# GewelsJI/MVLT

Hardware: AMD Instinct MI355X
Metric: image-text pairs/sec/node, PVT-tiny MVLT pre-train step (higher is better)
Workload: dtype bf16

## Files before the change

### mvlt_amd/_lib.py

```python
import ctypes as C
import os

import torch

_HERE = os.path.dirname(os.path.abspath(__file__))
LIB_PATH = os.environ.get("MVLT_HIP_LIB") or os.path.join(_HERE, "libmvlt_hip.so")


class MVLTError(RuntimeError):
    pass


if not os.path.exists(LIB_PATH):
    raise ImportError(f"{LIB_PATH} is missing: build it with `python -m mvlt_amd.build` (hipcc, gfx950). "
                      "mvlt_amd has no CPU or eager fallback.")
lib = C.CDLL(LIB_PATH)

c_int, c_float, c_void_p, c_long = C.c_int, C.c_float, C.c_void_p, C.c_long


class RowMap(C.Structure):
    _fields_ = [(n, c_int) for n in ("mode", "rows_per_batch", "batch_stride", "offset",
                                     "r", "w_in", "tokens_in", "hw_out", "w_out", "c_seg", "h_in")]

# ... 225 lines not shown

PLAN_VERSION = 3
_plan_sizes = [(n, getattr(lib, n + "_sizeof")(), C.sizeof(c)) for n, c in PLAN_STRUCTS]
if lib.mvlt_plan_version() != PLAN_VERSION or any(have != want for _, have, want in _plan_sizes):
    raise ImportError(f"plan entry points mismatch: {LIB_PATH} is version {lib.mvlt_plan_version()}, the binding is version {PLAN_VERSION}; (struct, bytes in the library, "
                      f"bytes in the binding): {_plan_sizes} (stale build? run python -m mvlt_amd.build)")

OPT_PROTOTYPES = {
    "mvlt_opt_version": (_i, []),
    "mvlt_adamw_step_groups": (_i, [_vp, _vp, _vp, _vp, _vp, _l, _vp, _vp, _vp, _i, _vp, _vp, _vp]),
}
for _name, (_res, _args) in OPT_PROTOTYPES.items():
    if not hasattr(lib, _name):
        raise ImportError(f"{LIB_PATH} does not export {_name} (include/mvlt_hip_opt.h): stale build? run python -m mvlt_amd.build")
    _fn = getattr(lib, _name)
    _fn.restype, _fn.argtypes = _res, _args

OPT_VERSION = 1
if lib.mvlt_opt_version() != OPT_VERSION:
    raise ImportError(f"optimizer entry points mismatch: {LIB_PATH} is version {lib.mvlt_opt_version()}, the binding is version {OPT_VERSION} (stale build? run python -m mvlt_amd.build)")

LAMB_PROTOTYPES = {
    "mvlt_lamb_version": (_i, []),
    "mvlt_lamb_check_tables": (_i, [_vp, _i, _vp, _i, _l, _i]),
    "mvlt_lamb_moments": (_i, [_vp, _vp, _vp, _vp, _l, _vp, _vp, _i, _vp, _i, _vp, _i, _vp, _vp, _vp, _vp]),
    "mvlt_lamb_fold": (_i, [_vp, _i, _vp, _i, _vp, _i, _i, _vp, _vp, _vp]),
    "mvlt_lamb_apply": (_i, [_vp, _vp, _vp, _vp, _l, _vp, _vp, _i, _vp, _i, _vp, _i, _vp, _vp, _vp]),
}
for _name, (_res, _args) in LAMB_PROTOTYPES.items():
    if not hasattr(lib, _name):
        raise ImportError(f"{LIB_PATH} does not export {_name} (include/mvlt_hip_lamb.h): stale build? run python -m mvlt_amd.build")
    _fn = getattr(lib, _name)
    _fn.restype, _fn.argtypes = _res, _args

LAMB_VERSION = 1
if lib.mvlt_lamb_version() != LAMB_VERSION:
    raise ImportError(f"LAMB entry points mismatch: {LIB_PATH} is version {lib.mvlt_lamb_version()}, the binding is version {LAMB_VERSION} (stale build? run python -m mvlt_amd.build)")

LOSS_PROTOTYPES = {
    "mvlt_loss_version": (_i, []),
    "mvlt_ce_smooth_fwd": (_i, [_vp, _vp, _l, _f, _vp, _vp, _vp, _vp, _i, _i, _i, _i, _vp]),
    "mvlt_ce_smooth_bwd": (_i, [_vp, _vp, _l, _f, _vp, _vp, _vp, _vp, _vp, _i, _i, _i, _i, _i, _i, _vp]),
}
for _name, (_res, _args) in LOSS_PROTOTYPES.items():
    if not hasattr(lib, _name):
        raise ImportError(f"{LIB_PATH} does not export {_name} (include/mvlt_hip_loss.h): stale build? run python -m mvlt_amd.build")
    _fn = getattr(lib, _name)
    _fn.restype, _fn.argtypes = _res, _args

LOSS_VERSION = 1
if lib.mvlt_loss_version() != LOSS_VERSION:
    raise ImportError(f"loss entry points mismatch: {LIB_PATH} is version {lib.mvlt_loss_version()}, the binding is version {LOSS_VERSION} (stale build? run python -m mvlt_amd.build)")

DT = {torch.bfloat16: 0, torch.float32: 1}


def last_kernel():
    s = lib.mvlt_last_kernel().decode()
    s = s.replace("(anonymous namespace)::", "")
    if s.startswith("void "):
        s = s[5:]
    depth = 0
    for i, ch in enumerate(s):
        depth += ch == "<"
        depth -= ch == ">"
        if ch == "(" and depth == 0:
            return s[:i]
    return s


def check(rc, what):
    if rc != 0:
        raise MVLTError(f"{what} failed ({rc}): {lib.mvlt_last_error().decode()}")


_raw_stream, _cur_device = torch._C._cuda_getCurrentRawStream, torch._C._cuda_getDevice


def stream_ptr():
    return _raw_stream(_cur_device())


def ptr(t):
    if t is None:
        return None
    if not t.is_cuda:
        raise MVLTError("mvlt_amd ops need CUDA/HIP tensors (no CPU fallback)")
    return t.data_ptr()


def rowmap(rows_per_batch=0, batch_stride=0, offset=0):
    return RowMap(0, rows_per_batch, batch_stride, offset, 0, 0, 0, 0, 0, 0, 0)


def patchmap(r, w_in, tokens_in, hw_out, w_out, c_seg):
    return RowMap(1, 0, 0, 0, r, w_in, tokens_in, hw_out, w_out, c_seg, 0)


def conv3map(h, w, tokens_in, c_seg):
    return RowMap(2, 0, 0, 0, 3, w, tokens_in, h * w, w, c_seg, h)
```

### mvlt_amd/build.py

```python
import concurrent.futures
import os
import subprocess
import sys

HERE = os.path.dirname(os.path.abspath(__file__))
CSRC = os.path.join(HERE, "csrc")
OBJ = os.path.join(HERE, "csrc", "_obj")
LIB = os.path.join(HERE, "libmvlt_hip.so")
ARCH = "gfx950"
FLAGS = ["--offload-arch=" + ARCH, "-O3", "-std=c++17", "-fPIC", "-ffp-contract=fast", "-Wno-unused-result"]
EXTRA = {f: ["-fno-slp-vectorize"] for f in ("mlp_fused.hip", "mlp_pipe.hip", "mlp_wgrad.hip")}


def _sources():
    return sorted(f for f in os.listdir(CSRC) if f.endswith(".hip"))


def source_hash():
    import hashlib
    h = hashlib.sha256()
    files = sorted(os.path.join(CSRC, f) for f in os.listdir(CSRC) if f.endswith((".hip", ".h", ".inc")))
    files += [os.path.join(HERE, "..", "include", h) for h in ("mvlt_hip.h", "mvlt_hip_ext.h", "mvlt_hip_ema.h", "mvlt_hip_plan.h", "mvlt_hip_opt.h", "mvlt_hip_lamb.h", "mvlt_hip_loss.h")]
    for f in files:
        h.update(os.path.basename(f).encode())
        h.update(open(f, "rb").read())
    return h.hexdigest()[:16]


def _deps_mtime():
    hdrs = [os.path.join(CSRC, f) for f in os.listdir(CSRC) if f.endswith((".h", ".inc"))]
    hdrs += [os.path.join(HERE, "..", "include", h) for h in ("mvlt_hip.h", "mvlt_hip_ext.h", "mvlt_hip_ema.h", "mvlt_hip_plan.h", "mvlt_hip_opt.h", "mvlt_hip_lamb.h", "mvlt_hip_loss.h")]
    return max(os.path.getmtime(h) for h in hdrs)


def _compile(src, force, verbose):
    s = os.path.join(CSRC, src)
    o = os.path.join(OBJ, src[:-4] + ".o")
    if not force and os.path.exists(o) and os.path.getmtime(o) >= max(os.path.getmtime(s), _deps_mtime()):
        return o
    cmd = ["hipcc", *FLAGS, *EXTRA.get(src, []), "-c", s, "-o", o]
    if verbose:
        print(" ".join(cmd), flush=True)
    r = subprocess.run(cmd, capture_output=True, text=True)
    if r.returncode != 0:
        raise RuntimeError(f"hipcc failed for {src}:\n{r.stdout}\n{r.stderr}")
    return o


def build(force=False, verbose=False):
    os.makedirs(OBJ, exist_ok=True)
    srcs = _sources()
    with concurrent.futures.ThreadPoolExecutor(max_workers=min(8, len(srcs))) as ex:
        objs = list(ex.map(lambda s: _compile(s, force, verbose), srcs))
    if force or not os.path.exists(LIB) or any(os.path.getmtime(o) > os.path.getmtime(LIB) for o in objs):
        cmd = ["hipcc", "--offload-arch=" + ARCH, "-shared", "-fPIC", *objs, "-o", LIB]
        if verbose:
            print(" ".join(cmd), flush=True)
        r = subprocess.run(cmd, capture_output=True, text=True)
        if r.returncode != 0:
            raise RuntimeError(f"link failed:\n{r.stdout}\n{r.stderr}")
    return LIB


if __name__ == "__main__":
    print(build(force="--force" in sys.argv, verbose="--verbose" in sys.argv or True))
```

### mvlt_amd/mim.py

```python
import torch

from . import layers, ops
from .layers import StoreAccess, _empty, linear, linear_bwd
from .params import pool_zeros
from .plan import plan_unit
from ._lib import conv3map, rowmap

BN_EPS, BN_MOM = 1e-5, 0.1
STAT_COPIES = 16
CONVS = ("reduction1", "reduction2", "reduction3", "conv_upsample1", "conv_upsample2", "conv_upsample3", "conv_upsample4",
         "conv_upsample5", "conv_concat2", "conv_concat3", "conv4")
_NO_BN_FOLD = False


def _z(shape, dev, dtype=torch.float32):
    return pool_zeros(shape, dtype, dev)


class MimStep(StoreAccess):
    def __init__(self, model, x2, x3, x4, sides, training, need_grad):
        self.m, self.S = model, model.store
        self.dt = model.compute_dtype
        self.dev = x2.device
        self.x = (x2, x3, x4)
        self.B = x2.shape[0]
        self.s1, self.s2, self.s3 = sides
        self.M1, self.M2, self.M3 = (self.B * h * w for h, w in sides)
        self.training = training
        self.need_grad = need_grad
        self.rec = {}
        self.nbt = []

    def conv_bn(self, name, xin, tokens_in, side, cin, cout, M):
        S, dev = self.S, self.dev
        p = f"t2i_head.{name}"
        amap = conv3map(side[0], side[1], tokens_in, cin)
        bn = getattr(self.m.t2i_head, name)[1]
        if not self.training and not self.need_grad and not _NO_BN_FOLD:
            r = dict(name=name, p=p, fold=self._folded(name, p, bn, cin, cout), xin=xin, amap=amap, cin=cin, cout=cout, M=M)
            self.rec[name] = r
            return r
        z16 = self.training and self.dt == torch.bfloat16
        z = _empty((M, cout), torch.float16 if z16 else torch.float32, dev)
        st = _z((2, STAT_COPIES, cout), dev) if self.training else (None, None)
        linear(xin, self.wK(p + ".0.weight"), z, M, a_map=amap, col_sum=st[0], col_sumsq=st[1], col_copies=STAT_COPIES)
        fin = None
        if self.training:
            mean, rstd = _empty((cout,), torch.float32, dev), _empty((cout,), torch.float32, dev)
            if z16 and cout % 8 == 0 and cout <= 256:
                fin = (st[0], st[1], bn.running_mean, bn.running_var)
            else:
                ops.bn_finalize(st[0], st[1], M, cout, BN_EPS, BN_MOM, mean, rstd, bn.running_mean, bn.running_var, copies=STAT_COPIES)
            self.nbt.append(bn.num_batches_tracked)
        else:
            mean = bn.running_mean
            rstd = torch.rsqrt(bn.running_var + BN_EPS)
        r = dict(name=name, p=p, z=z, mean=mean, rstd=rstd, xin=xin, amap=amap, cin=cin, cout=cout, M=M, side=side,
                 tokens_in=tokens_in, fin=fin)
        self.rec[name] = r
        return r

    def _folded(self, name, p, bn, cin, cout):
        S, m = self.S, self.m
        key = (S.refresh_count, bn.running_mean._version, bn.running_var._version, bn.num_batches_tracked._version, self.dt)
        cache = m.__dict__.setdefault("_mim_fold", {})
        hit = cache.get(name)
        if hit is None or hit[0] != key:
            scale = self.f32(p + ".1.weight") * torch.rsqrt(bn.running_var.float() + BN_EPS)
            shift = (self.f32(p + ".1.bias") - bn.running_mean.float() * scale).contiguous()
            wk = (self.f32(p + ".0.weight").permute(0, 2, 3, 1).reshape(cout, 9 * cin) * scale[:, None]).to(self.dt).contiguous()
            hit = cache[name] = (key, wk, shift)
        return hit[1], hit[2]

    def norm(self, r, y32=None, ld32=0, y16=None, ld16=0):
        if "fold" in r:
            wk, shift = r["fold"]
            for y in (y32, y16):
                if y is not None:
                    linear(r["xin"], wk, y, r["M"], a_map=r["amap"], bias=shift)
            return
        if r.get("fin") is not None:
            s1, s2, rm, rv = r["fin"]
            r["fin"] = None
            ops.bn_finalize_norm(r["z"], r["cout"], s1, s2, STAT_COPIES, BN_EPS, BN_MOM, r["mean"], r["rstd"], rm, rv, self.f32(r["p"] + ".1.weight"),
                                 self.f32(r["p"] + ".1.bias"), r["M"], r["cout"], y32, ld32, y16, ld16)
            return
        ops.bn_norm(r["z"], r["cout"], r["mean"], r["rstd"], self.f32(r["p"] + ".1.weight"), self.f32(r["p"] + ".1.bias"), r["M"], r["cout"],
                    y32, ld32, y16, ld16)

    def up2(self, x32, ldx, side, C, out=None, ldo=None):
        B = self.B
        if out is None:
            out, ldo = _empty((B * 4 * side[0] * side[1], C), self.dt, self.dev), C
        ops.upsample_fwd(x32, ldx, B, side[0], side[1], C, 2, out, ldo)
        return out

    def forward(self, target=None):
        S, dev, dt, B = self.S, self.dev, self.dt, self.B
        x2, x3, x4 = self.x
        s1, s2, s3, M1, M2, M3 = self.s1, self.s2, self.s3, self.M1, self.M2, self.M3
        C2, C3, C4 = x2.shape[2], x3.shape[2], x4.shape[2]
        ch = 64
        f = self.rec
        f16 = torch.float16 if (self.training and dt == torch.bfloat16) else torch.float32
        r = self.conv_bn("reduction1", x2, x2.shape[1], s1, C2, ch, M1); low = _empty((M1, ch), f16, dev); self.norm(r, low, ch)
        r = self.conv_bn("reduction2", x3, x3.shape[1], s2, C3, ch, M2); mid = _empty((M2, ch), torch.float32, dev); self.norm(r, mid, ch)
        r = self.conv_bn("reduction3", x4, x4.shape[1], s3, C4, ch, M3); high = _empty((M3, ch), torch.float32, dev); self.norm(r, high, ch)
        uph = self.up2(high, ch, s3, ch)
        HW1, HW2 = s1[0] * s1[1], s2[0] * s2[1]
        cat2 = _empty((M2, 2 * ch), dt, dev)
        r = self.conv_bn("conv_upsample1", uph, HW2, s2, ch, ch, M2); cu1o = _empty((M2, ch), torch.float32, dev); self.norm(r, cu1o, ch)
        a = _empty((M2, ch), torch.float32, dev)
        ops.ew_mul(a, ch, cu1o, ch, mid, ch, M=M2, Cdim=ch, out16=cat2, ld16=2 * ch)
        r = self.conv_bn("conv_upsample4", uph, HW2, s2, ch, ch, M2); self.norm(r, y16=cat2[:, ch:], ld16=2 * ch)
        r = self.conv_bn("conv_concat2", cat2, HW2, s2, 2 * ch, 2 * ch, M2); c = _empty((M2, 2 * ch), torch.float32, dev); self.norm(r, c, 2 * ch)
        cat3 = _empty((M1, 3 * ch), dt, dev)
        upm = self.up2(mid, ch, s2, ch)
        r = self.conv_bn("conv_upsample2", upm, HW1, s1, ch, ch, M1); cu2o = _empty((M1, ch), f16, dev); self.norm(r, cu2o, ch)
        upa = self.up2(a, ch, s2, ch)
        r = self.conv_bn("conv_upsample3", upa, HW1, s1, ch, ch, M1); cu3o = _empty((M1, ch), f16, dev); self.norm(r, cu3o, ch)
        ops.ew_mul(None, 0, cu2o, ch, cu3o, ch, low, ch, M=M1, Cdim=ch, out16=cat3, ld16=3 * ch)
        upc = self.up2(c, 2 * ch, s2, 2 * ch)
        r = self.conv_bn("conv_upsample5", upc, HW1, s1, 2 * ch, 2 * ch, M1); self.norm(r, y16=cat3[:, ch:], ld16=3 * ch)
        d16 = _empty((M1, 3 * ch), dt, dev)
        r = self.conv_bn("conv_concat3", cat3, HW1, s1, 3 * ch, 3 * ch, M1); self.norm(r, y16=d16, ld16=3 * ch)
        e16 = _empty((M1, 3 * ch), dt, dev)
        r = self.conv_bn("conv4", d16, HW1, s1, 3 * ch, 3 * ch, M1); self.norm(r, y16=e16, ld16=3 * ch)
        sc = _empty((M1, 3), torch.float32, dev)
        linear(e16, S.extra["t2i_head.score.0.weight::W"], sc, bias=self.f32("t2i_head.score.0.bias"))
        if target is not None:
            acc = pool_zeros((1,), torch.float32, dev)
            ops.upsample_l1_fwd(sc, 3, B, s1[0], s1[1], 3, 8, target, acc)
            out = (acc / target.numel()).reshape(())
            self.sc, self.target = sc, target
        else:
            out = _empty((B, 3, 8 * s1[0], 8 * s1[1]), torch.float32, dev)
            ops.upsample_fwd(sc, 3, B, s1[0], s1[1], 3, 8, out, 0, nchw=True)
        if self.nbt:
            torch._foreach_add_(self.nbt, 1)
            self.nbt = []
        if self.need_grad:
            self.keep = dict(low=low, mid=mid, cu1o=cu1o, cu2o=cu2o, cu3o=cu3o, e16=e16)
        else:
            self.rec = {}
        return out

    def bn_conv_bwd(self, name, dy, lddy, dx=None, accumulate=False, dx_map=None, dx_dtype=torch.float32, need_dx=True):
        S, dev, dt = self.S, self.dev, self.dt
        r = self.rec[name]
        p, M, cin, cout = r["p"], r["M"], r["cin"], r["cout"]
        red = _z((2, cout), dev)
        ops.bn_bwd_reduce(dy, lddy, r["z"], cout, r["mean"], r["rstd"], M, cout, red[0], red[1])
        dz = _empty((M, cout), dt, dev)
        ops.bn_bwd_apply(dy, lddy, r["z"], cout, r["mean"], r["rstd"], self.f32(p + ".1.weight"), red[0], red[1], M, cout, dz, cout,
                         g_beta=self.g(p + ".1.bias"), g_gamma=self.g(p + ".1.weight"))
        layers.conv_wgrad(S, p + ".0.weight", dz, r["xin"], r["amap"])
        if not need_dx:
            return None
        gmap = conv3map(r["side"][0], r["side"][1], r["side"][0] * r["side"][1], cout)
        if dx is None:
            dx = _empty((M, cin), dx_dtype, dev)
        linear(dz, S.extra[p + ".0.weight::F"], dx, M, a_map=gmap, c_map=dx_map, R=dx if accumulate else None)
        return dx

    def backward(self, dout, sink=None, dgrad=True):
        S, dev, dt, B = self.S, self.dev, self.dt, self.B
        s1, s2, s3, M1, M2, M3 = self.s1, self.s2, self.s3, self.M1, self.M2, self.M3
        ch = 64
        k = self.keep
        dsc_p = _z((M1, 8), dev, dt)
        if getattr(self, "target", None) is not None:
            ops.upsample_l1_bwd(self.sc, 3, B, s1[0], s1[1], 3, 8, self.target, dout.reshape(1).float().contiguous(), dsc_p, 8)
            self.sc = self.target = None
        else:
            dout = dout.contiguous().float()
            ops.upsample_bwd(dout, 0, True, B, s1[0], s1[1], 3, 8, dsc_p, 8)
        gd = dt if dt == torch.bfloat16 else torch.float32
        de = _empty((M1, 3 * ch), gd, dev)
        linear_bwd(True, dsc_p, k["e16"], self.g("t2i_head.score.0.weight"), self.g("t2i_head.score.0.bias"), self.wT("t2i_head.score.0.weight"), de)
        dd = self.bn_conv_bwd("conv4", de, 3 * ch, dx_dtype=gd)
        dcat3 = self.bn_conv_bwd("conv_concat3", dd, 3 * ch, dx_dtype=gd)
        dupc = self.bn_conv_bwd("conv_upsample5", dcat3[:, ch:], 3 * ch, dx_dtype=gd)
        dc = _empty((M2, 2 * ch), torch.float32, dev)
        ops.upsample_bwd(dupc, 2 * ch, False, B, s2[0], s2[1], 2 * ch, 2, dc, 2 * ch)
        db = dcat3
        dcu2o, dcu3o, dlow = _empty((M1, ch), gd, dev), _empty((M1, ch), gd, dev), _empty((M1, ch), gd, dev)
        ops.ew_mul3_bwd(db, 3 * ch, k["cu2o"], k["cu3o"], k["low"], ch, dcu2o, dcu3o, dlow, M1, ch)
        dcat2 = _z((M2, 2 * ch), dev)
        dupa = self.bn_conv_bwd("conv_upsample3", dcu3o, ch, dx_dtype=gd)
        ops.upsample_bwd(dupa, ch, False, B, s2[0], s2[1], ch, 2, dcat2, 2 * ch, accumulate=True)
        dupm = self.bn_conv_bwd("conv_upsample2", dcu2o, ch, dx_dtype=gd)
        dmid = _empty((M2, ch), torch.float32, dev)
        ops.upsample_bwd(dupm, ch, False, B, s2[0], s2[1], ch, 2, dmid, ch)
        self.bn_conv_bwd("conv_concat2", dc, 2 * ch, dx=dcat2, accumulate=True)
        duph = self.bn_conv_bwd("conv_upsample4", dcat2[:, ch:], 2 * ch)
        dcu1o = _empty((M2, ch), torch.float32, dev)
        ops.ew_mul(dcu1o, ch, dcat2, 2 * ch, k["mid"], ch, M=M2, Cdim=ch)
        ops.ew_mul(dmid, ch, dcat2, 2 * ch, k["cu1o"], ch, M=M2, Cdim=ch, accumulate=True)
        self.bn_conv_bwd("conv_upsample1", dcu1o, ch, dx=duph, accumulate=True)
        dhigh = _empty((M3, ch), torch.float32, dev)
        ops.upsample_bwd(duph, ch, False, B, s3[0], s3[1], ch, 2, dhigh, ch)
        grads = []
        for name, dy, x, side in (("reduction1", dlow, self.x[0], s1), ("reduction2", dmid, self.x[1], s2), ("reduction3", dhigh, self.x[2], s3)):
            if not dgrad:
                self.bn_conv_bwd(name, dy, ch, need_dx=False)
                grads.append(None)
                continue
            if name == "reduction3" and sink is not None:
                dxs, ret = sink.take(x.shape, x.dtype, x.device)
            else:
                dxs = ret = S.own(torch.empty_like(x))
                dxs[:, side[0] * side[1]:].zero_()
            self.bn_conv_bwd(name, dy, ch, dx=dxs, dx_map=rowmap(side[0] * side[1], x.shape[1], 0))
            grads.append(ret)
        self.rec, self.keep = {}, {}
        return grads


class _MimFn(torch.autograd.Function):
    @staticmethod
    def forward(ctx, x2, x3, x4, model, sides, need_grad, sink=None, target=None):
        step = MimStep(model, x2, x3, x4, sides, model.training, need_grad)
        out = step.forward(target)
        ctx.step, ctx.sink = step, sink
        ctx.dgrad = plan_unit(model, "t2i_head").dgrad
        return out

    @staticmethod
    def backward(ctx, dout):
        step = ctx.step
        step.S.queue_finalize()
        g2, g3, g4 = step.backward(dout, ctx.sink, ctx.dgrad)
        ctx.step = ctx.sink = None
        step.S.fold_copies(early=True)
        step.S.announce_prefix("t2i_head.")
        return g2, g3, g4, None, None, None, None, None


def mim_head(model, x2, x3, x4, sides, need_grad, sink=None, target=None):
    return _MimFn.apply(x2, x3, x4, model, sides, need_grad, sink, target)
```

### mvlt_amd/ops.py

```python
import ctypes as C

import torch

from . import _lib as L
from ._lib import DT, check, patchmap, ptr, rowmap, stream_ptr

_ID = rowmap()


def _gemm_nt_args(A, B, C_out, M, N, K, lda, ldb, ldc, *, a_map=None, c_map=None, bias=None, act=0, H=None,
                  row_scale=None, rows_per_scale=0, R=None, col_sum=None, col_sumsq=None, col_copies=0, split_k=0, post_ln=None):
    assert A.dtype == B.dtype and A.dtype in DT and (C_out.dtype in DT or (C_out.dtype == torch.float16 and col_sum is not None))
    if bias is not None:
        assert bias.dtype == torch.float32
    if row_scale is not None:
        assert row_scale.dtype == torch.float32
    if R is not None:
        assert R.dtype == C_out.dtype or (R.dtype == torch.float32 and C_out.dtype == torch.bfloat16)
    if H is not None:
        assert H.dtype == C_out.dtype
    if col_sum is not None:
        assert col_sum.dtype == torch.float32 and col_sumsq is not None and col_sumsq.dtype == torch.float32
    a = L.GemmNTArgs(A=ptr(A), B=ptr(B), C=ptr(C_out), M=M, N=N, K=K, lda=lda, ldb=ldb, ldc=ldc,
                     dtype=DT[A.dtype], out_dtype=2 if C_out.dtype == torch.float16 else DT[C_out.dtype], a_map=a_map or _ID, c_map=c_map or _ID,
# ... 379 lines not shown
def cast_bf16(src, dst, n):
    check(L.lib.mvlt_cast_bf16(ptr(src), ptr(dst), n, stream_ptr()), "mvlt_cast_bf16")


def row_scale(x, scale, rows_per_scale, M, Cdim, out):
    assert x.is_contiguous() and out.is_contiguous() and scale.dtype == torch.float32 and x.dtype == out.dtype
    check(L.lib.mvlt_row_scale(ptr(x), ptr(scale), rows_per_scale, M, Cdim, ptr(out), DT[x.dtype], stream_ptr()), "mvlt_row_scale")


def transpose_cast(w, out, R, Ccols, ld_out):
    assert w.dtype == torch.float32 and w.is_contiguous()
    check(L.lib.mvlt_transpose_cast(ptr(w), ptr(out), R, Ccols, ld_out, DT[out.dtype], stream_ptr()), "mvlt_transpose_cast")


ZDT = {torch.float32: 1, torch.float16: 2}


def col_stats(z, ldz, M, Cdim, s, ss):
    check(L.lib.mvlt_col_stats(ptr(z), ldz, M, Cdim, ptr(s), ptr(ss), stream_ptr()), "mvlt_col_stats")


def bn_finalize(s, ss, M, Cdim, eps, momentum, mean, rstd, running_mean=None, running_var=None, copies=1):
    check(L.lib.mvlt_bn_finalize(ptr(s), ptr(ss), copies, M, Cdim, eps, momentum, ptr(mean), ptr(rstd), ptr(running_mean), ptr(running_var), stream_ptr()),
          "mvlt_bn_finalize")


def bn_norm(z, ldz, mean, rstd, gamma, beta, M, Cdim, y32=None, ld32=0, y16=None, ld16=0):
    check(L.lib.mvlt_bn_norm(ptr(z), ldz, ZDT[z.dtype], ptr(mean), ptr(rstd), ptr(gamma), ptr(beta), M, Cdim, ptr(y32), ld32, ZDT[y32.dtype] if y32 is not None else 1, ptr(y16), ld16,
                             DT[y16.dtype] if y16 is not None else 0, stream_ptr()), "mvlt_bn_norm")


def bn_finalize_norm(z, ldz, s, ss, copies, eps, momentum, mean, rstd, running_mean, running_var, gamma, beta, M, Cdim, y32=None, ld32=0, y16=None, ld16=0):
    assert z.dtype == torch.float16 and (y16 is None or y16.dtype == torch.bfloat16)
    check(L.lib.mvlt_bn_finalize_norm(ptr(z), ldz, ptr(s), ptr(ss), copies, eps, momentum, ptr(mean), ptr(rstd), ptr(running_mean), ptr(running_var), ptr(gamma), ptr(beta), M, Cdim,
                                      ptr(y32), ld32, ZDT[y32.dtype] if y32 is not None else 1, ptr(y16), ld16, stream_ptr()), "mvlt_bn_finalize_norm")


def bn_bwd_reduce(dy, lddy, z, ldz, mean, rstd, M, Cdim, s1, s2):
    assert dy.dtype in DT and z.dtype in ZDT
    check(L.lib.mvlt_bn_bwd_reduce(ptr(dy), lddy, ptr(z), ldz, ZDT[z.dtype], ptr(mean), ptr(rstd), M, Cdim, ptr(s1), ptr(s2), DT[dy.dtype], stream_ptr()), "mvlt_bn_bwd_reduce")


def bn_bwd_apply(dy, lddy, z, ldz, mean, rstd, gamma, s1, s2, M, Cdim, dz16, lddz, g_beta=None, g_gamma=None):
    assert dy.dtype in DT and z.dtype in ZDT
    check(L.lib.mvlt_bn_bwd_apply(ptr(dy), lddy, ptr(z), ldz, ZDT[z.dtype], ptr(mean), ptr(rstd), ptr(gamma), ptr(s1), ptr(s2), M, Cdim, ptr(dz16), lddz,
                                  ptr(g_beta), ptr(g_gamma), DT[dz16.dtype], DT[dy.dtype], stream_ptr()), "mvlt_bn_bwd_apply")


def ew_mul3_bwd(dy, lddy, a, b, c, ld, da, db, dc, M, Cdim):
    assert dy.dtype in DT and da.dtype == db.dtype == dc.dtype == dy.dtype and a.dtype == b.dtype == c.dtype and a.dtype in ZDT
    check(L.lib.mvlt_ew_mul3_bwd(ptr(dy), lddy, ptr(a), ptr(b), ptr(c), ld, ZDT[a.dtype], ptr(da), ptr(db), ptr(dc), M, Cdim, DT[dy.dtype], stream_ptr()), "mvlt_ew_mul3_bwd")


def ew_mul(out, ldo, a, lda, b, ldb, c=None, ldc=0, *, M, Cdim, accumulate=False, out16=None, ld16=0):
    assert a.dtype == b.dtype and (c is None or c.dtype == a.dtype) and a.dtype in ZDT
    check(L.lib.mvlt_ew_mul(ptr(out), ldo, ptr(a), lda, ptr(b), ldb, ptr(c), ldc, ZDT[a.dtype], M, Cdim, 1 if accumulate else 0, ptr(out16), ld16,
                            DT[out16.dtype] if out16 is not None else 0, stream_ptr()), "mvlt_ew_mul")


def upsample_fwd(x, ldx, B, H, W, Cdim, scale, out, ldo, nchw=False):
    check(L.lib.mvlt_upsample_fwd(ptr(x), ldx, B, H, W, Cdim, scale, ptr(out), ldo, DT[out.dtype], 1 if nchw else 0, stream_ptr()), "mvlt_upsample_fwd")


def upsample_bwd(dy, lddy, nchw, B, H, W, Cdim, scale, dx, lddx, accumulate=False):
    assert dy.dtype in DT and dx.dtype in DT
    check(L.lib.mvlt_upsample_bwd(ptr(dy), lddy, 1 if nchw else 0, B, H, W, Cdim, scale, ptr(dx), lddx, 1 if accumulate else 0, DT[dx.dtype],
                                  DT[dy.dtype], stream_ptr()), "mvlt_upsample_bwd")


def upsample_l1_ok(W, scale):
    return W <= 64 and (W * scale) % 4 == 0 and W * scale <= 256


def upsample_l1_fwd(x, ldx, B, H, W, Cdim, scale, target, loss_sum):
    assert x.dtype == target.dtype == loss_sum.dtype == torch.float32 and target.is_contiguous()
    check(L.lib.mvlt_upsample_l1_fwd(ptr(x), ldx, B, H, W, Cdim, scale, ptr(target), ptr(loss_sum), stream_ptr()), "mvlt_upsample_l1_fwd")


def upsample_l1_bwd(x, ldx, B, H, W, Cdim, scale, target, gscale, dx, lddx):
    assert x.dtype == target.dtype == gscale.dtype == torch.float32 and dx.dtype in DT and target.is_contiguous()
    check(L.lib.mvlt_upsample_l1_bwd(ptr(x), ldx, B, H, W, Cdim, scale, ptr(target), ptr(gscale), ptr(dx), lddx, DT[dx.dtype], stream_ptr()),
          "mvlt_upsample_l1_bwd")


def _mlp_fwd_args(x, w1, b1, w2, b2, residual, out, M, Cdim, hid, *, row_scale=None, rows_per_scale=0, h_out=None, ln=None, out_op=None, post_ln=None):
    assert w1.dtype == torch.bfloat16 and w2.dtype == torch.bfloat16
    assert residual.dtype == torch.float32 and residual.is_contiguous() and (out is not None or out_op is not None)
    assert out is None or out.dtype == torch.float32
    assert out_op is None or (out_op.dtype == torch.bfloat16 and out_op.is_contiguous())
    a = L.MlpArgs(x=ptr(x), w1=ptr(w1), wb=ptr(w2), b1=ptr(b1), b2=ptr(b2), residual=ptr(residual), row_scale=ptr(row_scale), rows_per_scale=rows_per_scale,
                  out=ptr(out), h_out=ptr(h_out), M=M, C=Cdim, hid=hid, out_op=ptr(out_op))
    if ln is None:
        assert x.dtype == torch.bfloat16
    else:
        g, b, eps, y, mean, rstd = ln
        assert g.dtype == b.dtype == mean.dtype == rstd.dtype == torch.float32 and y.dtype == torch.bfloat16 and y.is_contiguous()
        a.ln_x, a.ln_gamma, a.ln_beta, a.ln_eps, a.ln_y, a.ln_mean, a.ln_rstd = ptr(residual), ptr(g), ptr(b), eps, ptr(y), ptr(mean), ptr(rstd)
    if post_ln is not None:
        pg, pb, peps, py, pm, pr = post_ln
        assert pg.dtype == pb.dtype == pm.dtype == pr.dtype == torch.float32 and py.dtype == torch.bfloat16 and py.is_contiguous()
        a.post_gamma, a.post_beta, a.post_eps, a.post_y, a.post_mean, a.post_rstd = ptr(pg), ptr(pb), peps, ptr(py), ptr(pm), ptr(pr)
    return a


def mlp_fwd(x, w1, b1, w2, b2, residual, out, *dims, out_op=None, **kw):
    check(L.lib.mvlt_mlp_fwd(C.byref(_mlp_fwd_args(x, w1, b1, w2, b2, residual, out, *dims, out_op=out_op, **kw)), stream_ptr()), "mvlt_mlp_fwd")
# ... 129 lines not shown
```

Baseline: 13470.

## Fuse MIM three-factor BN-normalize product and its backward with BN reductions

Adds HIP kernels that apply batch-norm finalize and normalize to three 64-channel factors (conv_upsample2, conv_upsample3, reduction1), multiply them, and write straight into the concat buffer. The backward computes the three factor gradients and the BN backward reductions in one pass, so the separate bn_bwd_reduce calls are skipped. This is meant to remove several intermediate fp16 tensors, extra kernel launches and repeated reads of the pre-norm activations in the t2i head. In exchange, every forward block recomputes the BN statistics from the per-copy sums, and backward needs an extra fold kernel over a scratch buffer.

Result: no change. 13510 (median of 6 runs) (+0.3%).

```diff
diff --git a/include/mvlt_hip_mim.h b/include/mvlt_hip_mim.h
--- /dev/null
+++ b/include/mvlt_hip_mim.h
@@ -0,0 +1,22 @@
+#ifndef MVLT_HIP_MIM_H
+#define MVLT_HIP_MIM_H
+#ifdef __cplusplus
+extern "C" {
+#endif
+
+#define MVLT_MIM_VERSION 1
+int mvlt_mim_version(void);
+
+int mvlt_mim_prod3_fwd(const void* const z[3] , int ldz, const float* const sum[3], const float* const sumsq[3], int copies, float eps, float momentum,
+                       float* const mean[3], float* const rstd[3], float* const running_mean[3], float* const running_var[3], const float* const gamma[3],
+                       const float* const beta[3], long M, int C, void* out , int ldo, void* stream);
+
+long mvlt_mim_prod3_bwd_scratch(long M, int C);
+int mvlt_mim_prod3_bwd(const void* dy , int lddy, const void* const z[3] , int ldz, const float* const mean[3], const float* const rstd[3],
+                       const float* const gamma[3], const float* const beta[3], long M, int C, void* const dfac[3] , float* scratch,
+                       float* const s1[3], float* const s2[3], void* stream);
+
+#ifdef __cplusplus
+}
+#endif
+#endif
diff --git a/mvlt_amd/_lib.py b/mvlt_amd/_lib.py
--- a/mvlt_amd/_lib.py
+++ b/mvlt_amd/_lib.py
@@ -301,6 +301,22 @@
 if lib.mvlt_loss_version() != LOSS_VERSION:
     raise ImportError(f"loss entry points mismatch: {LIB_PATH} is version {lib.mvlt_loss_version()}, the binding is version {LOSS_VERSION} (stale build? run python -m mvlt_amd.build)")
 
+MIM_PROTOTYPES = {
+    "mvlt_mim_version": (_i, []),
+    "mvlt_mim_prod3_fwd": (_i, [_vp, _i, _vp, _vp, _i, _f, _f, _vp, _vp, _vp, _vp, _vp, _vp, _l, _i, _vp, _i, _vp]),
+    "mvlt_mim_prod3_bwd_scratch": (_l, [_l, _i]),
+    "mvlt_mim_prod3_bwd": (_i, [_vp, _i, _vp, _i, _vp, _vp, _vp, _vp, _l, _i, _vp, _vp, _vp, _vp, _vp]),
+}
+for _name, (_res, _args) in MIM_PROTOTYPES.items():
+    if not hasattr(lib, _name):
+        raise ImportError(f"{LIB_PATH} does not export {_name} (include/mvlt_hip_mim.h): stale build? run python -m mvlt_amd.build")
+    _fn = getattr(lib, _name)
+    _fn.restype, _fn.argtypes = _res, _args
+
+MIM_VERSION = 1
+if lib.mvlt_mim_version() != MIM_VERSION:
+    raise ImportError(f"MIM entry points mismatch: {LIB_PATH} is version {lib.mvlt_mim_version()}, the binding is version {MIM_VERSION} (stale build? run python -m mvlt_amd.build)")
+
 DT = {torch.bfloat16: 0, torch.float32: 1}
 
 
diff --git a/mvlt_amd/build.py b/mvlt_amd/build.py
--- a/mvlt_amd/build.py
+++ b/mvlt_amd/build.py
@@ -20,7 +20,7 @@
     import hashlib
     h = hashlib.sha256()
     files = sorted(os.path.join(CSRC, f) for f in os.listdir(CSRC) if f.endswith((".hip", ".h", ".inc")))
-    files += [os.path.join(HERE, "..", "include", h) for h in ("mvlt_hip.h", "mvlt_hip_ext.h", "mvlt_hip_ema.h", "mvlt_hip_plan.h", "mvlt_hip_opt.h", "mvlt_hip_lamb.h", "mvlt_hip_loss.h")]
+    files += [os.path.join(HERE, "..", "include", h) for h in ("mvlt_hip.h", "mvlt_hip_ext.h", "mvlt_hip_ema.h", "mvlt_hip_plan.h", "mvlt_hip_opt.h", "mvlt_hip_lamb.h", "mvlt_hip_loss.h", "mvlt_hip_mim.h")]
     for f in files:
         h.update(os.path.basename(f).encode())
         h.update(open(f, "rb").read())
@@ -29,7 +29,7 @@
 
 def _deps_mtime():
     hdrs = [os.path.join(CSRC, f) for f in os.listdir(CSRC) if f.endswith((".h", ".inc"))]
-    hdrs += [os.path.join(HERE, "..", "include", h) for h in ("mvlt_hip.h", "mvlt_hip_ext.h", "mvlt_hip_ema.h", "mvlt_hip_plan.h", "mvlt_hip_opt.h", "mvlt_hip_lamb.h", "mvlt_hip_loss.h")]
+    hdrs += [os.path.join(HERE, "..", "include", h) for h in ("mvlt_hip.h", "mvlt_hip_ext.h", "mvlt_hip_ema.h", "mvlt_hip_plan.h", "mvlt_hip_opt.h", "mvlt_hip_lamb.h", "mvlt_hip_loss.h", "mvlt_hip_mim.h")]
     return max(os.path.getmtime(h) for h in hdrs)
 
 
diff --git a/mvlt_amd/csrc/mim_fused.hip b/mvlt_amd/csrc/mim_fused.hip
--- /dev/null
+++ b/mvlt_amd/csrc/mim_fused.hip
@@ -0,0 +1,275 @@
+#include "common.h"
+#include "../../include/mvlt_hip.h"
+#include "../../include/mvlt_hip_mim.h"
+
+namespace {
+
+constexpr int NT = 256;
+constexpr int PC = 64;
+constexpr int BROWS = NT / 64 * 8;
+constexpr int BU = 2;
+constexpr int BWGS = 512;
+constexpr int FOLD_NT = 1024;
+
+typedef _Float16 f16x8 __attribute__((ext_vector_type(8)));
+
+__device__ __forceinline__ void load8(const float* p, float (&v)[8]) {
+  const f32x4 a = *(const f32x4*)p, b = *(const f32x4*)(p + 4);
+#pragma unroll
+  for (int e = 0; e < 4; ++e) { v[e] = a[e]; v[4 + e] = b[e]; }
+}
+__device__ __forceinline__ void store8(bf16* p, const bf16x8& o) { st_g<MVLT_NT_MIM>((bf16x8*)p, o); }
+
+struct Prod3Fwd {
+  const _Float16* z[3];
+  const float* sum[3];
+  const float* sumsq[3];
+  float* mean[3];
+  float* rstd[3];
+  float* running_mean[3];
+  float* running_var[3];
+  const float* gamma[3];
+  const float* beta[3];
+};
+
+__global__ __launch_bounds__(NT) void mim_prod3_fwd_kernel(Prod3Fwd a, int ldz, int copies, long Mstat, float eps, float momentum, long M, bf16* out, int ldo) {
+  __shared__ __attribute__((aligned(16))) float s_mu[3][PC], s_rs[3][PC], s_ga[3][PC], s_be[3][PC];
+#pragma unroll
+  for (int k = 0; k < 3; ++k) {
+    for (int c = threadIdx.x; c < PC; c += NT) {
+      float m, r;
+      if (a.sum[k]) {
+        float s1 = 0.f, s2 = 0.f;
+        for (int j = 0; j < copies; ++j) { s1 += a.sum[k][(long)j * PC + c]; s2 += a.sumsq[k][(long)j * PC + c]; }
+        m = s1 / (int)Mstat;
+        const float var = fmaxf(s2 / (int)Mstat - m * m, 0.f);
+        r = rsqrtf(var + eps);
+        if (blockIdx.x == 0) {
+          a.mean[k][c] = m; a.rstd[k][c] = r;
+          if (a.running_mean[k]) {
+            a.running_mean[k][c] = (1.f - momentum) * a.running_mean[k][c] + momentum * m;
+            const float unb = Mstat > 1 ? var * ((float)(int)Mstat / (float)((int)Mstat - 1)) : var;
+            a.running_var[k][c] = (1.f - momentum) * a.running_var[k][c] + momentum * unb;
+          }
+        }
+      } else {
+        m = a.mean[k][c]; r = a.rstd[k][c];
+      }
+      s_mu[k][c] = m; s_rs[k][c] = r; s_ga[k][c] = a.gamma[k][c]; s_be[k][c] = a.beta[k][c];
+    }
+  }
+  __syncthreads();
+  constexpr int cq = PC / 8;
+  for (long i = (long)blockIdx.x * NT + threadIdx.x; i < M * cq; i += (long)gridDim.x * NT) {
+    const long r = i / cq; const int c = (int)(i - r * cq) * 8;
+    f16x8 zv[3];
+#pragma unroll
+    for (int k = 0; k < 3; ++k) zv[k] = *(const f16x8*)(a.z[k] + r * ldz + c);
+    float f[3][8];
+#pragma unroll
+    for (int k = 0; k < 3; ++k)
+#pragma unroll
+      for (int e = 0; e < 8; ++e) {
+        const float v = (float)zv[k][e];
+        const float o = (v - s_mu[k][c + e]) * s_rs[k][c + e] * s_ga[k][c + e] + s_be[k][c + e];
+        f[k][e] = (float)(_Float16)o;
+      }
+    bf16x8 o;
+#pragma unroll
+    for (int e = 0; e < 8; ++e) {
+      float p = f[0][e] * f[1][e];
+      p *= f[2][e];
+      o[e] = (bf16)p;
+    }
+    store8(out + r * ldo + c, o);
+  }
+}
+
+struct Prod3Bwd {
+  const _Float16* z[3];
+  const float* mean[3];
+  const float* rstd[3];
+  const float* gamma[3];
+  const float* beta[3];
+  bf16* d[3];
+};
+
+struct Prod3Stats { float mu[3][8], rs[3][8], ga[3][8], be[3][8]; };
+
+__device__ __forceinline__ void prod3_bwd_row(const bf16x8& g8, const f16x8 (&zv)[3], const Prod3Stats& s, bf16* const (&d)[3], long off, float (&a1)[3][8], float (&a2)[3][8]) {
+  float f[3][8], zc[3][8];
+#pragma unroll
+  for (int k = 0; k < 3; ++k)
+#pragma unroll
+    for (int e = 0; e < 8; ++e) {
+      const float v = (float)zv[k][e];
+      const float o = (v - s.mu[k][e]) * s.rs[k][e] * s.ga[k][e] + s.be[k][e];
+      f[k][e] = (float)(_Float16)o;
+      zc[k][e] = v - s.mu[k][e];
+    }
+  bf16x8 o[3];
+#pragma unroll
+  for (int e = 0; e < 8; ++e) {
+    const float g = (float)g8[e];
+    o[0][e] = (bf16)(g * f[1][e] * f[2][e]);
+    o[1][e] = (bf16)(g * f[0][e] * f[2][e]);
+    o[2][e] = (bf16)(g * f[0][e] * f[1][e]);
+  }
+#pragma unroll
+  for (int k = 0; k < 3; ++k) {
+    store8(d[k] + off, o[k]);
+#pragma unroll
+    for (int e = 0; e < 8; ++e) {
+      const float dv = (float)o[k][e];
+      a1[k][e] += dv;
+      a2[k][e] += dv * zc[k][e] * s.rs[k][e];
+    }
+  }
+}
+
+__global__ __launch_bounds__(NT) void mim_prod3_bwd_kernel(const bf16* dy, int lddy, Prod3Bwd a, int ldz, long M, float* partial, int rows_per_wg) {
+  __shared__ float sm[NT / 64][6][PC];
+  const int lane = threadIdx.x & 63, wave = threadIdx.x >> 6;
+  const int tc = (lane & 7) * 8, tr = wave * 8 + (lane >> 3);
+  Prod3Stats s;
+#pragma unroll
+  for (int k = 0; k < 3; ++k) { load8(a.mean[k] + tc, s.mu[k]); load8(a.rstd[k] + tc, s.rs[k]); load8(a.gamma[k] + tc, s.ga[k]); load8(a.beta[k] + tc, s.be[k]); }
+  float a1[3][8], a2[3][8];
+#pragma unroll
+  for (int k = 0; k < 3; ++k)
+#pragma unroll
+    for (int e = 0; e < 8; ++e) { a1[k][e] = 0.f; a2[k][e] = 0.f; }
+  bf16* const d[3] = {a.d[0], a.d[1], a.d[2]};
+  const long r0 = (long)blockIdx.x * rows_per_wg;
+  const long r1 = (r0 + rows_per_wg < M) ? r0 + rows_per_wg : M;
+  long r = r0 + tr;
+  for (; r + (long)(BU - 1) * BROWS < r1; r += (long)BU * BROWS) {
+    bf16x8 g8[BU];
+    f16x8 zv[BU][3];
+#pragma unroll
+    for (int u = 0; u < BU; ++u) {
+      const long ru = r + (long)u * BROWS;
+      g8[u] = *(const bf16x8*)(dy + ru * lddy + tc);
+#pragma unroll
+      for (int k = 0; k < 3; ++k) zv[u][k] = *(const f16x8*)(a.z[k] + ru * ldz + tc);
+    }
+#pragma unroll
+    for (int u = 0; u < BU; ++u) prod3_bwd_row(g8[u], zv[u], s, d, (r + (long)u * BROWS) * PC + tc, a1, a2);
+  }
+  for (; r < r1; r += BROWS) {
+    const bf16x8 g8 = *(const bf16x8*)(dy + r * lddy + tc);
+    f16x8 zv[3];
+#pragma unroll
+    for (int k = 0; k < 3; ++k) zv[k] = *(const f16x8*)(a.z[k] + r * ldz + tc);
+    prod3_bwd_row(g8, zv, s, d, r * PC + tc, a1, a2);
+  }
+#pragma unroll
+  for (int o = 8; o < 64; o <<= 1)
+#pragma unroll
+    for (int k = 0; k < 3; ++k)
+#pragma unroll
+      for (int e = 0; e < 8; ++e) { a1[k][e] += __shfl_xor(a1[k][e], o); a2[k][e] += __shfl_xor(a2[k][e], o); }
+  if (lane < 8) {
+#pragma unroll
+    for (int k = 0; k < 3; ++k)
+#pragma unroll
+      for (int e = 0; e < 8; ++e) { sm[wave][2 * k][tc + e] = a1[k][e]; sm[wave][2 * k + 1][tc + e] = a2[k][e]; }
+  }
+  __syncthreads();
+  for (int i = threadIdx.x; i < 6 * PC; i += NT) {
+    const int j = i / PC, c = i - j * PC;
+    float t = sm[0][j][c];
+#pragma unroll
+    for (int w = 1; w < NT / 64; ++w) t += sm[w][j][c];
+    partial[(long)blockIdx.x * 6 * PC + i] = t;
+  }
+}
+
+struct Prod3Sums { float* s[6]; };
+
+__global__ __launch_bounds__(FOLD_NT) void mim_prod3_fold_kernel(const float* partial, int nwg, Prod3Sums out) {
+  __shared__ float sm[FOLD_NT / PC][PC];
+  const int j = blockIdx.x, c = threadIdx.x & (PC - 1), g = threadIdx.x / PC;
+  float t = 0.f;
+#pragma unroll 8
+  for (int w = g; w < nwg; w += FOLD_NT / PC) t += partial[((long)w * 6 + j) * PC + c];
+  sm[g][c] = t;
+  __syncthreads();
+  if (g == 0) {
+    float v = sm[0][c];
+#pragma unroll
+    for (int i = 1; i < FOLD_NT / PC; ++i) v += sm[i][c];
+    float* dst = j == 0 ? out.s[0] : j == 1 ? out.s[1] : j == 2 ? out.s[2] : j == 3 ? out.s[3] : j == 4 ? out.s[4] : out.s[5];
+    dst[c] = v;
+  }
+}
+
+inline bool al16(const void* q) { return ((uintptr_t)q & 15) == 0; }
+
+inline void bwd_geometry(long M, int* rows_per_wg, int* grid) {
+  constexpr int step = BROWS * BU;
+  long rows = (M + BWGS - 1) / BWGS;
+  rows = (rows + step - 1) / step * step;
+  *rows_per_wg = (int)rows;
+  *grid = (int)((M + rows - 1) / rows);
+}
+
+}
+
+extern "C" int mvlt_mim_version(void) { return MVLT_MIM_VERSION; }
+
+extern "C" int mvlt_mim_prod3_fwd(const void* const z[3], int ldz, const float* const sum[3], const float* const sumsq[3], int copies, float eps, float momentum,
+                                  float* const mean[3], float* const rstd[3], float* const running_mean[3], float* const running_var[3], const float* const gamma[3],
+                                  const float* const beta[3], long M, int C, void* out, int ldo, void* stream) {
+  MVLT_REQUIRE(z && sum && sumsq && mean && rstd && running_mean && running_var && gamma && beta && out, "mvlt_mim_prod3_fwd: null pointer");
+  MVLT_REQUIRE(C == PC, "mvlt_mim_prod3_fwd: C = %d, the factors have 64 channels", C);
+  MVLT_REQUIRE(M < (1L << 31) && copies >= 1, "mvlt_mim_prod3_fwd: M below 2^31, copies >= 1");
+  MVLT_REQUIRE(ldz >= C && ldz % 8 == 0 && ldo >= C && ldo % 8 == 0 && al16(out), "mvlt_mim_prod3_fwd: row strides are multiples of 8 and >= C, out 16-byte aligned");
+  Prod3Fwd a;
+  for (int k = 0; k < 3; ++k) {
+    MVLT_REQUIRE(z[k] && mean[k] && rstd[k] && gamma[k] && beta[k], "mvlt_mim_prod3_fwd: null pointer (factor %d)", k);
+    MVLT_REQUIRE((sum[k] == nullptr) == (sumsq[k] == nullptr), "mvlt_mim_prod3_fwd: sum and sumsq go together (factor %d)", k);
+    MVLT_REQUIRE((running_mean[k] == nullptr) == (running_var[k] == nullptr), "mvlt_mim_prod3_fwd: running_mean and running_var go together (factor %d)", k);
+    MVLT_REQUIRE(al16(z[k]), "mvlt_mim_prod3_fwd: z is 16-byte aligned (factor %d)", k);
+    a.z[k] = (const _Float16*)z[k]; a.sum[k] = sum[k]; a.sumsq[k] = sumsq[k]; a.mean[k] = mean[k]; a.rstd[k] = rstd[k];
+    a.running_mean[k] = sum[k] ? running_mean[k] : nullptr; a.running_var[k] = sum[k] ? running_var[k] : nullptr;
+    a.gamma[k] = gamma[k]; a.beta[k] = beta[k];
+  }
+  if (M <= 0) return MVLT_OK;
+  long g = (M * (PC / 8) + NT - 1) / NT;
+  if (g > 2048) g = 2048;
+  MVLT_LAUNCH(mim_prod3_fwd_kernel, dim3((int)g), dim3(NT), 0, (hipStream_t)stream, a, ldz, copies, M, eps, momentum, M, (bf16*)out, ldo);
+  return mvlt_check_launch("mvlt_mim_prod3_fwd");
+}
+
+extern "C" long mvlt_mim_prod3_bwd_scratch(long M, int C) {
+  if (M <= 0 || C != PC) return 0;
+  int rows_per_wg, grid;
+  bwd_geometry(M, &rows_per_wg, &grid);
+  return (long)grid * 6 * PC;
+}
+
+extern "C" int mvlt_mim_prod3_bwd(const void* dy, int lddy, const void* const z[3], int ldz, const float* const mean[3], const float* const rstd[3],
+                                  const float* const gamma[3], const float* const beta[3], long M, int C, void* const dfac[3], float* scratch,
+                                  float* const s1[3], float* const s2[3], void* stream) {
+  MVLT_REQUIRE(dy && z && mean && rstd && gamma && beta && dfac && scratch && s1 && s2, "mvlt_mim_prod3_bwd: null pointer");
+  MVLT_REQUIRE(C == PC, "mvlt_mim_prod3_bwd: C = %d, the factors have 64 channels", C);
+  MVLT_REQUIRE(M < (1L << 31), "mvlt_mim_prod3_bwd: M below 2^31");
+  MVLT_REQUIRE(ldz >= C && ldz % 8 == 0 && lddy >= C && lddy % 8 == 0 && al16(dy) && al16(scratch), "mvlt_mim_prod3_bwd: row strides are multiples of 8 and >= C, dy and scratch 16-byte aligned");
+  Prod3Bwd a;
+  Prod3Sums out;
+  for (int k = 0; k < 3; ++k) {
+    MVLT_REQUIRE(z[k] && mean[k] && rstd[k] && gamma[k] && beta[k] && dfac[k] && s1[k] && s2[k], "mvlt_mim_prod3_bwd: null pointer (factor %d)", k);
+    MVLT_REQUIRE(al16(z[k]) && al16(dfac[k]) && al16(mean[k]) && al16(rstd[k]) && al16(gamma[k]) && al16(beta[k]), "mvlt_mim_prod3_bwd: 16-byte aligned tensors (factor %d)", k);
+    a.z[k] = (const _Float16*)z[k]; a.mean[k] = mean[k]; a.rstd[k] = rstd[k]; a.gamma[k] = gamma[k]; a.beta[k] = beta[k]; a.d[k] = (bf16*)dfac[k];
+    out.s[2 * k] = s1[k]; out.s[2 * k + 1] = s2[k];
+  }
+  if (M <= 0) return MVLT_OK;
+  int rows_per_wg, grid;
+  bwd_geometry(M, &rows_per_wg, &grid);
+  MVLT_LAUNCH(mim_prod3_bwd_kernel, dim3(grid), dim3(NT), 0, (hipStream_t)stream, (const bf16*)dy, lddy, a, ldz, M, scratch, rows_per_wg);
+  int rc = mvlt_check_launch("mvlt_mim_prod3_bwd");
+  if (rc != MVLT_OK) return rc;
+  MVLT_LAUNCH(mim_prod3_fold_kernel, dim3(6), dim3(FOLD_NT), 0, (hipStream_t)stream, (const float*)scratch, grid, out);
+  return mvlt_check_launch("mvlt_mim_prod3_bwd");
+}
diff --git a/mvlt_amd/mim.py b/mvlt_amd/mim.py
--- a/mvlt_amd/mim.py
+++ b/mvlt_amd/mim.py
@@ -18,7 +18,7 @@
 
 
 class MimStep(StoreAccess):
-    def __init__(self, model, x2, x3, x4, sides, training, need_grad):
+    def __init__(self, model, x2, x3, x4, sides, training, need_grad, fuse_products=True):
         self.m, self.S = model, model.store
         self.dt = model.compute_dtype
         self.dev = x2.device
@@ -30,6 +30,7 @@
         self.need_grad = need_grad
         self.rec = {}
         self.nbt = []
+        self.fused = bool(fuse_products) and training and self.dt == torch.bfloat16
 
     def conv_bn(self, name, xin, tokens_in, side, cin, cout, M):
         S, dev = self.S, self.dev
@@ -88,6 +89,10 @@
         ops.bn_norm(r["z"], r["cout"], r["mean"], r["rstd"], self.f32(r["p"] + ".1.weight"), self.f32(r["p"] + ".1.bias"), r["M"], r["cout"],
                     y32, ld32, y16, ld16)
 
+    def _prod3(self):
+        rs = [self.rec[n] for n in ("conv_upsample2", "conv_upsample3", "reduction1")]
+        return rs, [self.f32(r["p"] + ".1.weight") for r in rs], [self.f32(r["p"] + ".1.bias") for r in rs]
+
     def up2(self, x32, ldx, side, C, out=None, ldo=None):
         B = self.B
         if out is None:
@@ -103,7 +108,10 @@
         ch = 64
         f = self.rec
         f16 = torch.float16 if (self.training and dt == torch.bfloat16) else torch.float32
-        r = self.conv_bn("reduction1", x2, x2.shape[1], s1, C2, ch, M1); low = _empty((M1, ch), f16, dev); self.norm(r, low, ch)
+        low = cu2o = cu3o = None
+        r = self.conv_bn("reduction1", x2, x2.shape[1], s1, C2, ch, M1)
+        if not self.fused:
+            low = _empty((M1, ch), f16, dev); self.norm(r, low, ch)
         r = self.conv_bn("reduction2", x3, x3.shape[1], s2, C3, ch, M2); mid = _empty((M2, ch), torch.float32, dev); self.norm(r, mid, ch)
         r = self.conv_bn("reduction3", x4, x4.shape[1], s3, C4, ch, M3); high = _empty((M3, ch), torch.float32, dev); self.norm(r, high, ch)
         uph = self.up2(high, ch, s3, ch)
@@ -116,10 +124,21 @@
         r = self.conv_bn("conv_concat2", cat2, HW2, s2, 2 * ch, 2 * ch, M2); c = _empty((M2, 2 * ch), torch.float32, dev); self.norm(r, c, 2 * ch)
         cat3 = _empty((M1, 3 * ch), dt, dev)
         upm = self.up2(mid, ch, s2, ch)
-        r = self.conv_bn("conv_upsample2", upm, HW1, s1, ch, ch, M1); cu2o = _empty((M1, ch), f16, dev); self.norm(r, cu2o, ch)
+        r = self.conv_bn("conv_upsample2", upm, HW1, s1, ch, ch, M1)
+        if not self.fused:
+            cu2o = _empty((M1, ch), f16, dev); self.norm(r, cu2o, ch)
         upa = self.up2(a, ch, s2, ch)
-        r = self.conv_bn("conv_upsample3", upa, HW1, s1, ch, ch, M1); cu3o = _empty((M1, ch), f16, dev); self.norm(r, cu3o, ch)
-        ops.ew_mul(None, 0, cu2o, ch, cu3o, ch, low, ch, M=M1, Cdim=ch, out16=cat3, ld16=3 * ch)
+        r = self.conv_bn("conv_upsample3", upa, HW1, s1, ch, ch, M1)
+        if self.fused:
+            rs, ga, be = self._prod3()
+            fin = [q["fin"] or (None, None, None, None) for q in rs]
+            ops.mim_prod3_fwd([q["z"] for q in rs], ch, [t[0] for t in fin], [t[1] for t in fin], STAT_COPIES, BN_EPS, BN_MOM, [q["mean"] for q in rs],
+                              [q["rstd"] for q in rs], [t[2] for t in fin], [t[3] for t in fin], ga, be, M1, ch, cat3, 3 * ch)
+            for q in rs:
+                q["fin"] = None
+        else:
+            cu3o = _empty((M1, ch), f16, dev); self.norm(r, cu3o, ch)
+            ops.ew_mul(None, 0, cu2o, ch, cu3o, ch, low, ch, M=M1, Cdim=ch, out16=cat3, ld16=3 * ch)
         upc = self.up2(c, 2 * ch, s2, 2 * ch)
         r = self.conv_bn("conv_upsample5", upc, HW1, s1, 2 * ch, 2 * ch, M1); self.norm(r, y16=cat3[:, ch:], ld16=3 * ch)
         d16 = _empty((M1, 3 * ch), dt, dev)
@@ -145,12 +164,13 @@
             self.rec = {}
         return out
 
-    def bn_conv_bwd(self, name, dy, lddy, dx=None, accumulate=False, dx_map=None, dx_dtype=torch.float32, need_dx=True):
+    def bn_conv_bwd(self, name, dy, lddy, dx=None, accumulate=False, dx_map=None, dx_dtype=torch.float32, need_dx=True, red=None):
         S, dev, dt = self.S, self.dev, self.dt
         r = self.rec[name]
         p, M, cin, cout = r["p"], r["M"], r["cin"], r["cout"]
-        red = _z((2, cout), dev)
-        ops.bn_bwd_reduce(dy, lddy, r["z"], cout, r["mean"], r["rstd"], M, cout, red[0], red[1])
+        if red is None:
+            red = _z((2, cout), dev)
+            ops.bn_bwd_reduce(dy, lddy, r["z"], cout, r["mean"], r["rstd"], M, cout, red[0], red[1])
         dz = _empty((M, cout), dt, dev)
         ops.bn_bwd_apply(dy, lddy, r["z"], cout, r["mean"], r["rstd"], self.f32(p + ".1.weight"), red[0], red[1], M, cout, dz, cout,
                          g_beta=self.g(p + ".1.bias"), g_gamma=self.g(p + ".1.weight"))
@@ -185,11 +205,18 @@
         ops.upsample_bwd(dupc, 2 * ch, False, B, s2[0], s2[1], 2 * ch, 2, dc, 2 * ch)
         db = dcat3
         dcu2o, dcu3o, dlow = _empty((M1, ch), gd, dev), _empty((M1, ch), gd, dev), _empty((M1, ch), gd, dev)
-        ops.ew_mul3_bwd(db, 3 * ch, k["cu2o"], k["cu3o"], k["low"], ch, dcu2o, dcu3o, dlow, M1, ch)
+        red3 = (None, None, None)
+        if self.fused:
+            rs, ga, be = self._prod3()
+            red3 = _empty((3, 2, ch), torch.float32, dev)
+            ops.mim_prod3_bwd(db, 3 * ch, [q["z"] for q in rs], ch, [q["mean"] for q in rs], [q["rstd"] for q in rs], ga, be, M1, ch, (dcu2o, dcu3o, dlow),
+                              _empty((ops.mim_prod3_bwd_scratch(M1, ch),), torch.float32, dev), [red3[i][0] for i in range(3)], [red3[i][1] for i in range(3)])
+        else:
+            ops.ew_mul3_bwd(db, 3 * ch, k["cu2o"], k["cu3o"], k["low"], ch, dcu2o, dcu3o, dlow, M1, ch)
         dcat2 = _z((M2, 2 * ch), dev)
-        dupa = self.bn_conv_bwd("conv_upsample3", dcu3o, ch, dx_dtype=gd)
+        dupa = self.bn_conv_bwd("conv_upsample3", dcu3o, ch, dx_dtype=gd, red=red3[1])
         ops.upsample_bwd(dupa, ch, False, B, s2[0], s2[1], ch, 2, dcat2, 2 * ch, accumulate=True)
-        dupm = self.bn_conv_bwd("conv_upsample2", dcu2o, ch, dx_dtype=gd)
+        dupm = self.bn_conv_bwd("conv_upsample2", dcu2o, ch, dx_dtype=gd, red=red3[0])
         dmid = _empty((M2, ch), torch.float32, dev)
         ops.upsample_bwd(dupm, ch, False, B, s2[0], s2[1], ch, 2, dmid, ch)
         self.bn_conv_bwd("conv_concat2", dc, 2 * ch, dx=dcat2, accumulate=True)
@@ -202,8 +229,9 @@
         ops.upsample_bwd(duph, ch, False, B, s3[0], s3[1], ch, 2, dhigh, ch)
         grads = []
         for name, dy, x, side in (("reduction1", dlow, self.x[0], s1), ("reduction2", dmid, self.x[1], s2), ("reduction3", dhigh, self.x[2], s3)):
+            red = red3[2] if name == "reduction1" else None
             if not dgrad:
-                self.bn_conv_bwd(name, dy, ch, need_dx=False)
+                self.bn_conv_bwd(name, dy, ch, need_dx=False, red=red)
                 grads.append(None)
                 continue
             if name == "reduction3" and sink is not None:
@@ -211,7 +239,7 @@
             else:
                 dxs = ret = S.own(torch.empty_like(x))
                 dxs[:, side[0] * side[1]:].zero_()
-            self.bn_conv_bwd(name, dy, ch, dx=dxs, dx_map=rowmap(side[0] * side[1], x.shape[1], 0))
+            self.bn_conv_bwd(name, dy, ch, dx=dxs, dx_map=rowmap(side[0] * side[1], x.shape[1], 0), red=red)
             grads.append(ret)
         self.rec, self.keep = {}, {}
         return grads
@@ -219,8 +247,8 @@
 
 class _MimFn(torch.autograd.Function):
     @staticmethod
-    def forward(ctx, x2, x3, x4, model, sides, need_grad, sink=None, target=None):
-        step = MimStep(model, x2, x3, x4, sides, model.training, need_grad)
+    def forward(ctx, x2, x3, x4, model, sides, need_grad, sink=None, target=None, fuse_products=True):
+        step = MimStep(model, x2, x3, x4, sides, model.training, need_grad, fuse_products)
         out = step.forward(target)
         ctx.step, ctx.sink = step, sink
         ctx.dgrad = plan_unit(model, "t2i_head").dgrad
@@ -234,8 +262,8 @@
         ctx.step = ctx.sink = None
         step.S.fold_copies(early=True)
         step.S.announce_prefix("t2i_head.")
-        return g2, g3, g4, None, None, None, None, None
-
-
-def mim_head(model, x2, x3, x4, sides, need_grad, sink=None, target=None):
-    return _MimFn.apply(x2, x3, x4, model, sides, need_grad, sink, target)
+        return g2, g3, g4, None, None, None, None, None, None
+
+
+def mim_head(model, x2, x3, x4, sides, need_grad, sink=None, target=None, fuse_products=True):
+    return _MimFn.apply(x2, x3, x4, model, sides, need_grad, sink, target, fuse_products)
diff --git a/mvlt_amd/ops.py b/mvlt_amd/ops.py
--- a/mvlt_amd/ops.py
+++ b/mvlt_amd/ops.py
@@ -455,6 +455,28 @@
     check(L.lib.mvlt_ew_mul3_bwd(ptr(dy), lddy, ptr(a), ptr(b), ptr(c), ld, ZDT[a.dtype], ptr(da), ptr(db), ptr(dc), M, Cdim, DT[dy.dtype], stream_ptr()), "mvlt_ew_mul3_bwd")
 
 
+def _ptr3(ts):
+    assert len(ts) == 3
+    return (C.c_void_p * 3)(*(ptr(t) for t in ts))
+
+
+def mim_prod3_fwd(z, ldz, s, ss, copies, eps, momentum, mean, rstd, running_mean, running_var, gamma, beta, M, Cdim, out, ldo):
+    assert all(t.dtype == torch.float16 for t in z) and out.dtype == torch.bfloat16
+    check(L.lib.mvlt_mim_prod3_fwd(_ptr3(z), ldz, _ptr3(s), _ptr3(ss), copies, eps, momentum, _ptr3(mean), _ptr3(rstd), _ptr3(running_mean), _ptr3(running_var),
+                                   _ptr3(gamma), _ptr3(beta), M, Cdim, ptr(out), ldo, stream_ptr()), "mvlt_mim_prod3_fwd")
+
+
+def mim_prod3_bwd_scratch(M, Cdim):
+    return L.lib.mvlt_mim_prod3_bwd_scratch(M, Cdim)
+
+
+def mim_prod3_bwd(dy, lddy, z, ldz, mean, rstd, gamma, beta, M, Cdim, dfac, scratch, s1, s2):
+    assert dy.dtype == torch.bfloat16 and all(t.dtype == torch.float16 for t in z) and all(t.dtype == torch.bfloat16 and t.is_contiguous() for t in dfac)
+    assert scratch.dtype == torch.float32 and scratch.numel() >= mim_prod3_bwd_scratch(M, Cdim)
+    check(L.lib.mvlt_mim_prod3_bwd(ptr(dy), lddy, _ptr3(z), ldz, _ptr3(mean), _ptr3(rstd), _ptr3(gamma), _ptr3(beta), M, Cdim, _ptr3(dfac), ptr(scratch),
+                                   _ptr3(s1), _ptr3(s2), stream_ptr()), "mvlt_mim_prod3_bwd")
+
+
 def ew_mul(out, ldo, a, lda, b, ldb, c=None, ldc=0, *, M, Cdim, accumulate=False, out16=None, ld16=0):
     assert a.dtype == b.dtype and (c is None or c.dtype == a.dtype) and a.dtype in ZDT
     check(L.lib.mvlt_ew_mul(ptr(out), ldo, ptr(a), lda, ptr(b), ldb, ptr(c), ldc, ZDT[a.dtype], M, Cdim, 1 if accumulate else 0, ptr(out16), ld16,
```
